# manuelruder/fast-artistic-videos

Measured on AMD Instinct MI355X. Metric: stylized frames/sec @1280x720, per-frame hot path (mask + warp + assembly + net + deprocess + PNG encode on the GPU) with inputs resident in HBM; file->PNG rate of the product CLI (BASELINE.json's end-to-end) in `end_to_end_fps` / `e2e`, PSNR vs CPU ref in `parity`, higher is better.
Workload: dtype f32

## Files before the change

### fast-artistic-videos_amd/csrc/conv_device.h

```cpp
#pragma once
#include "fav_internal.h"

namespace fav {

typedef float f32x16 __attribute__((ext_vector_type(16)));
typedef float v4f __attribute__((ext_vector_type(4)));
typedef int v4i __attribute__((ext_vector_type(4)));
typedef float v2f __attribute__((ext_vector_type(2)));

constexpr int BM = CONV_BM;
constexpr int BK = 32;
constexpr int LDSS = 36;
constexpr int SK_GRID = 512;

__device__ __forceinline__ int xcd_linear_block()
{
    const int nwg = gridDim.x, q = nwg >> 3, r = nwg & 7, xcd = blockIdx.x & 7, idx = blockIdx.x >> 3;
    return (xcd < r ? xcd * (q + 1) : r * (q + 1) + (xcd - r) * q) + idx;
}

__device__ __forceinline__ void store16_wt(void* p, v4f v)
{
    asm volatile("global_store_dwordx4 %0, %1, off sc1" ::"v"(p), "v"(v) : "memory");
}

__device__ __forceinline__ float2 merge_wave_stats(const float2* st, const int* wn, int NW, int pitch, int c, int* n_out)
{
    int n = 0; float s = 0.f;
    for (int w = 0; w < NW; ++w) { n += wn[w]; s += (float)wn[w] * st[w * pitch + c].x; }
    const float mean = n ? s / (float)n : 0.f;
    float m2 = 0.f;
    for (int w = 0; w < NW; ++w) { const float d = st[w * pitch + c].x - mean; m2 += st[w * pitch + c].y + (float)wn[w] * d * d; }
    *n_out = n;
    return make_float2(mean, m2);
}

__device__ __forceinline__ float4 affine4_lo(float4 v, const float* sc, const float* sh, float lo)
{
    const float4 s = *reinterpret_cast<const float4*>(sc);
    const float4 b = *reinterpret_cast<const float4*>(sh);
    v.x = fmaxf(fmaf(v.x, s.x, b.x), lo); v.y = fmaxf(fmaf(v.y, s.y, b.y), lo);
    v.z = fmaxf(fmaf(v.z, s.z, b.z), lo); v.w = fmaxf(fmaf(v.w, s.w, b.w), lo);
    return v;
}

__device__ __forceinline__ float4 affine4(float4 v, const float* sc, const float* sh, int relu)
{
    const float4 s = *reinterpret_cast<const float4*>(sc);
    const float4 b = *reinterpret_cast<const float4*>(sh);
    v.x = fmaf(v.x, s.x, b.x); v.y = fmaf(v.y, s.y, b.y); v.z = fmaf(v.z, s.z, b.z); v.w = fmaf(v.w, s.w, b.w);
    if (relu) { v.x = fmaxf(v.x, 0.f); v.y = fmaxf(v.y, 0.f); v.z = fmaxf(v.z, 0.f); v.w = fmaxf(v.w, 0.f); }
    return v;
// ... 4 lines not shown
```

### fast-artistic-videos_amd/csrc/fav_internal.h

```cpp
#pragma once
#include <hip/hip_runtime.h>
#include <cstdarg>
#include <cstdint>
#include <cstdio>
#include <exception>
#include <new>
#include <string>
#include <vector>

#include "../../include/fav.h"

#include <cstdlib>
inline const char* diag_env(const char* name)
{
#ifdef FAV_DIAG
    return getenv(name);
#else
    (void)name;
    return nullptr;
#endif
}

namespace fav {

// ... 71 lines not shown
__host__ __device__ inline bool stat_acc_poisoned(long long hi_sum, long long hi_squares)
{
    return hi_sum >= STAT_NONFINITE / 2 || hi_sum <= -(STAT_NONFINITE / 2) || hi_squares >= STAT_NONFINITE / 2 || hi_squares <= -(STAT_NONFINITE / 2);
}

struct ConvLaunch {
    const float* in = nullptr;
    int IH = 0, IW = 0;
    int IWp = 0;
    int ups = 0;
    int stuff = 0;
    int CIN = 0;
    Affine pre;
    const float* wgt = nullptr;
    const unsigned short* wgt16 = nullptr;
    const float* bias = nullptr;
    int COUT = 0, COUTp = 0;
    int KH = 0, KW = 0, stride = 1, pad = 0;
    int Kpad = 0;
    int OH = 0, OW = 0;
    float* out = nullptr;
    float* partials = nullptr;
    int final_mode = 0;
    float tanh_mul = 1.f;
    float* out_planar = nullptr;
    float* out_raw_nchw = nullptr;
    float* sk_ws = nullptr; unsigned* sk_flags = nullptr; unsigned sk_epoch = 0;
    unsigned* sk_err = nullptr;
    int reserve_cus = 0;
    int no_sk = 0;
    const float* join_skip = nullptr; float* join_out = nullptr; int OWp = 0;
    long long* stat_acc = nullptr;
    float* ks_ws = nullptr; int* ks_cnt = nullptr;
};
inline size_t conv3_wino4_ksplit_bytes() { return (size_t)256 * 2 * 256 * 128 * sizeof(float); }
size_t conv_streamk_workspace_bytes();
int conv_streamk_grid();
constexpr int CONV_BM = 128;
inline int conv_mblocks(int OH, int OW) { return (OH * OW + CONV_BM - 1) / CONV_BM; }
int launch_conv(const ConvLaunch& p, hipStream_t st);
bool conv_c8_eligible(int cin_pitch, int coutp, int k, int stride, int stages, int ups);
int conv_c8_tiles(int OH, int OW);
int launch_conv_c8(const ConvLaunch& p, int* counts, hipStream_t st);
bool conv_c8d_eligible(int cin_pitch, int cin_real, int coutp, int k, int stride, int stages, int ups);
void conv_c8d_pack(const float* w, int cin, int cout, std::vector<float>& out);
int launch_conv_c8d(const ConvLaunch& p, int cin_real, const float* wc8d, int* counts, hipStream_t st);
bool conv3_halo_eligible(int cin_pitch, int coutp, int k, int stride);
int conv3_halo_tiles(int OH, int OW, bool edge_b);
int launch_conv3_halo(const ConvLaunch& p, int* counts, hipStream_t st);
bool conv3s2_eligible(int cin_pitch, int coutp, int k, int stride, int stages, int ups);
int conv3s2_tiles(int OH, int OW);
int launch_conv3s2(const ConvLaunch& p, int* counts, hipStream_t st);
bool conv_fold_eligible(int cin_pitch, int cout, int k, int stride);
bool conv_fold_launchable(int cin_pitch, int k, int pad, int ups, int IH, int IW);
int launch_conv_fold(const ConvLaunch& p, const float* wfold, hipStream_t st);
int conv_first_tiles(int OH, int OW);
int launch_conv_first(const ConvLaunch& p, int cin_real, const float* wpk, int* counts, hipStream_t st);
bool conv_first2d_eligible(int cin_pitch, int cin_real, int coutp, int k, int stride, int stages, int ups);
int conv_first2d_tiles(int OH, int OW);
int launch_conv_first2d(const ConvLaunch& p, int cin_real, const float* wpk, int* counts, hipStream_t st);
bool conv3_wino_eligible(int cin_pitch, int cout, int coutp, int k, int stride, int pad, int stages, int ups);
int conv3_wino_tiles(int OH, int OW);
int launch_conv3_wino(const ConvLaunch& p, const float* wpk, int* counts, hipStream_t st);
bool conv3_wino4_eligible(int cin_pitch, int cout, int coutp, int k, int stride, int pad, int stages, int ups);
int conv3_wino4_tiles(int OH, int OW);
int launch_conv3_wino4(const ConvLaunch& p, const float* wpk, int* counts, hipStream_t st);
// ... 106 lines not shown
```

### fast-artistic-videos_amd/csrc/kernels_first.hip

```cpp
#include <algorithm>
#include <cstdlib>
#include <vector>

#include "fav_internal.h"
#include "conv_device.h"
#include "launch_common.h"
#include "first_pack.h"
#include "first2d_pack.h"

namespace fav {

namespace {

constexpr int F_TH = 8, F_TW = 64;
constexpr int F_HR = F_TH + 8, F_HC = F_TW + 8;
constexpr int F_HALF = F_HC / 2;
constexpr int F_RP = F_HC;
constexpr int F_CPL = F_HR * F_RP;
constexpr int F_HP = F_HR * F_HC;
constexpr int F_NH = (F_HP + 511) / 512;

struct FirstArgs {
    const float* in; const float* wpk; const float* bias;
    float* out; float2* partials; int* counts;
    int IH, IW, IWp, COUT, pad, OH, OW, tiles_x, tiles_y;
    int COUTP, groups;
    long long* dbg = nullptr;
};

__device__ __forceinline__ float2 merge_rows(const float2* st, const int* wn, int c, int* n_out)
{
    int n = 0; float s = 0.f;
    for (int w = 0; w < 8; ++w) { n += wn[w]; s += (float)wn[w] * st[w * 32 + c].x; }
    const float mean = n ? s / (float)n : 0.f;
    float m2 = 0.f;
    for (int w = 0; w < 8; ++w) { const float d = st[w * 32 + c].x - mean; m2 += st[w * 32 + c].y + (float)wn[w] * d * d; }
    *n_out = n;
    return make_float2(mean, m2);
}

constexpr int f_off(int e) { return (e & 1) * F_HALF + (e >> 1); }

template <int CR>
__global__ __launch_bounds__(512, 2) void conv_first_kernel(const FirstArgs p)
{
    constexpr int NCC = (CR / 2) * 27, NJ = NCC + 14, LAST = CR - 1;
    extern __shared__ __attribute__((aligned(16))) float smem[];
    float* const Ws = smem;
    float* const Hs = Ws + 4 * NJ * 64;
    float* const red = Hs + CR * F_CPL;
    const int t = threadIdx.x, lane = t & 63, wave = t >> 6;

    for (int e = t; e < 4 * NJ * 16; e += 512) *reinterpret_cast<v4f*>(Ws + e * 4) = *reinterpret_cast<const v4f*>(p.wpk + e * 4);

    const int ntiles = p.tiles_x * p.tiles_y;
    float4 hlo[F_NH], hhi[F_NH];
#define FL_LOAD_HALO(tile_)                                                                         \
    {                                                                                               \
        const int ty_ = (tile_) / p.tiles_x, tx_ = (tile_) - ty_ * p.tiles_x;                       \
// ... 146 lines not shown
    }
#undef FL_LOAD_HALO
#undef FL_STORE_HALO
}

template <int CR>
int launch_first_t(const FirstArgs& a, int reserve_cus, hipStream_t st)
{
    const size_t lds = (size_t)(4 * conv_first_pairs(CR) * 64 + CR * F_CPL + 8 * 64 + 8) * sizeof(float);
    static PerDevice cache; int cus;
    FAV_HIP(launch_cus(cache, &cus, conv_first_kernel<CR>));
    const int tiles = a.tiles_x * a.tiles_y;
    const int grid = persistent_slots(cus, reserve_cus);
    hipLaunchKernelGGL((conv_first_kernel<CR>), dim3(tiles < grid ? tiles : grid), dim3(512), lds, st, a);
    FAV_LAUNCH_CHECK("conv_first_kernel");
    return FAV_OK;
}


constexpr int G_TH = 16, G_TW = 32;
constexpr int G_HR = G_TH + 8, G_HC = G_TW + 8;
constexpr int G_CPL = G_HR * G_HC + 16;
constexpr int G_HP = G_HR * G_HC;
constexpr int G_NH = (G_HP + 511) / 512;

template <int CR, bool WIDE = false>
__global__ __launch_bounds__(512, 2) void conv_first2d_kernel(const FirstArgs p)
{
    constexpr int NQ = (9 * CR + 3) / 4;
    extern __shared__ __attribute__((aligned(16))) float smem[];
    float* const Ws = smem;
    float* const Hs = Ws + 16 * NQ * 128;
    float* const red = Hs + CR * G_CPL;
    const int t = threadIdx.x, lane = t & 63, wave = t >> 6;

    const int grp = WIDE ? blockIdx.x % p.groups : 0, tstep = WIDE ? gridDim.x / p.groups : gridDim.x;
    const int PITCH = WIDE ? p.COUTP : 32;
    const float* const wsrc = p.wpk + (WIDE ? (size_t)grp * (16 * NQ * 128) : 0);
    for (int e = t; e < 16 * NQ * 32; e += 512) *reinterpret_cast<v4f*>(Ws + e * 4) = *reinterpret_cast<const v4f*>(wsrc + e * 4);

    const int ntiles = p.tiles_x * p.tiles_y;
    float4 hlo[G_NH], hhi[G_NH];
    const __amdgpu_buffer_rsrc_t irs = __builtin_amdgcn_make_buffer_rsrc(const_cast<float*>(p.in), 0, p.IH * p.IWp * 32, 0x00020000);
#define G_LOAD_HALO(tile_)                                                                          \
    {                                                                                               \
        const bool tv_ = (tile_) < ntiles;                                                          \
        const int ty_ = (tile_) / p.tiles_x, tx_ = (tile_) - ty_ * p.tiles_x;                       \
        _Pragma("unroll") for (int i = 0; i < G_NH; ++i) {                                          \
            const int pix_ = min(t + 512 * i, G_HP - 1), hy_ = pix_ / G_HC, hx_ = pix_ - hy_ * G_HC; \
            const int iy_ = ty_ * G_TH - p.pad + hy_, ix_ = tx_ * G_TW - p.pad + hx_;               \
            const bool v_ = tv_ & ((unsigned)iy_ < (unsigned)p.IH) & ((unsigned)ix_ < (unsigned)p.IW); \
            const int off_ = v_ ? (iy_ * p.IWp + ix_) * 32 : (int)0xFFFFFF00;                       \
            hlo[i] = __builtin_bit_cast(float4, __builtin_amdgcn_raw_buffer_load_b128(irs, off_, 0, 0));          \
            hhi[i] = CR > 4 ? __builtin_bit_cast(float4, __builtin_amdgcn_raw_buffer_load_b128(irs, off_ + 16, 0, 0)) : make_float4(0.f, 0.f, 0.f, 0.f); \
        }                                                                                           \
    }
#define G_STORE_HALO()                                                                              \
    {                                                                                               \
        _Pragma("unroll") for (int i = 0; i < G_NH; ++i) {                                          \
            float* d_ = Hs + min(t + 512 * i, G_HP - 1);                                            \
            const float c_[8] = {hlo[i].x, hlo[i].y, hlo[i].z, hlo[i].w, hhi[i].x, hhi[i].y, hhi[i].z, hhi[i].w}; \
            _Pragma("unroll") for (int c = 0; c < CR; ++c) d_[c * G_CPL] = c_[c];                   \
        }                                                                                           \
    }

    int tile = WIDE ? blockIdx.x / p.groups : blockIdx.x;
    G_LOAD_HALO(tile);
    G_STORE_HALO();

    const int txl = lane & 15, g = lane >> 4;
    int qoff[NQ];
#pragma unroll
    for (int q = 0; q < NQ; ++q) {
        const int idx = 4 * q + g;
        const int c = idx / 9, a = (idx - 9 * c) / 3, b = idx - 9 * c - 3 * a;
        qoff[q] = idx < 9 * CR ? c * G_CPL + 3 * a * G_HC + 3 * b : 0;
    }
    const float* const a_lane = Hs + 2 * wave * G_HC + 2 * txl;
    const float* const b_lo = Ws + lane;
    int hi_words = 8 * NQ * 128;
    asm volatile("" : "+v"(hi_words));
    const float* const b_hi = b_lo + hi_words;
    __syncthreads();

#ifdef FAV_DIAG
    long long dt_[5] = {0, 0, 0, 0, 0}, tq_ = 0; int ntl_ = 0;
#define G_DBG(i_) { if (p.dbg && t == 0) { const long long n_ = wall_clock64(); dt_[i_] += n_ - tq_; tq_ = n_; } }
    if (p.dbg && t == 0) tq_ = wall_clock64();
#else
#define G_DBG(i_)
#endif
    for (; tile < ntiles; tile += tstep) {
        const int nxt = tile + tstep;
        G_LOAD_HALO(nxt);
        G_DBG(0);
        v4f acc[16][2];
#pragma unroll
        for (int ps = 0; ps < 16; ++ps)
#pragma unroll
            for (int nt = 0; nt < 2; ++nt) acc[ps][nt] = v4f{0.f, 0.f, 0.f, 0.f};

        float R[2][16], B[2][8];
#define G_READ_R(set_, q_)                                                                          \
        { const float* rb_ = a_lane + qoff[q_];                                                     \
          _Pragma("unroll") for (int r = 0; r < 4; ++r) _Pragma("unroll") for (int d = 0; d < 4; ++d) R[set_][4 * r + d] = rb_[r * G_HC + d]; }
#define G_READ_B(set_, q_, i_)                                                                      \
        { _Pragma("unroll") for (int j = 0; j < 4; ++j) _Pragma("unroll") for (int nt = 0; nt < 2; ++nt) \
              B[set_][2 * j + nt] = ((i_) < 2 ? b_lo : b_hi)[(((4 * ((i_) & 1) + j) * NQ + (q_)) * 2 + nt) * 64]; }
#define G_FENCE() __builtin_amdgcn_sched_barrier(0)
        G_READ_R(0, 0);
        G_READ_B(0, 0, 0);
#pragma unroll
        for (int q = 0; q < NQ; ++q) {
            if (q + 1 < NQ) { G_READ_R((q + 1) & 1, q + 1); }
#pragma unroll
            for (int i = 0; i < 4; ++i) {
                float L[4], V[4];
                const float* Rq = R[q & 1];
#pragma unroll
                for (int d = 0; d < 4; ++d)
                    L[d] = i == 0 ? Rq[d] - Rq[8 + d] : i == 1 ? Rq[4 + d] + Rq[8 + d] : i == 2 ? Rq[8 + d] - Rq[4 + d] : Rq[4 + d] - Rq[12 + d];
                V[0] = L[0] - L[2]; V[1] = L[1] + L[2]; V[2] = L[2] - L[1]; V[3] = L[1] - L[3];
                const int nset = (4 * q + i + 1) & 1;
                if (i < 3) { G_READ_B(nset, q, i + 1); } else if (q + 1 < NQ) { G_READ_B(nset, q + 1, 0); }
                G_FENCE();
                const float* Bq = B[(4 * q + i) & 1];
// ... 10 lines not shown
#undef G_FENCE
        G_DBG(1);
        __syncthreads();
        G_STORE_HALO();
        G_DBG(2);

        const int ty = tile / p.tiles_x, tx = tile - ty * p.tiles_x;
        const int oy0 = ty * G_TH + 2 * __builtin_amdgcn_readfirstlane(wave), ox0 = tx * G_TW;
        const bool inside = oy0 + 2 <= p.OH && ox0 + G_TW <= p.OW && grp * 32 + 32 <= p.COUT;
        float y[2][4][2][2];
        float sm[2] = {0.f, 0.f};
#pragma unroll
        for (int nt = 0; nt < 2; ++nt) {
            const int ch = grp * 32 + nt * 16 + txl;
            const float bv = p.bias[ch];
            const v2f bv2 = v2f{bv, bv};
#pragma unroll
            for (int rp = 0; rp < 4; rp += 2) {
                v2f Q[4][2];
#pragma unroll
                for (int i = 0; i < 4; ++i) {
                    const v2f m0 = rp ? acc[4 * i][nt].zw : acc[4 * i][nt].xy, m1 = rp ? acc[4 * i + 1][nt].zw : acc[4 * i + 1][nt].xy;
                    const v2f m2 = rp ? acc[4 * i + 2][nt].zw : acc[4 * i + 2][nt].xy, m3 = rp ? acc[4 * i + 3][nt].zw : acc[4 * i + 3][nt].xy;
                    Q[i][0] = (m0 + m1) + m2; Q[i][1] = (m1 - m2) - m3;
                }
#pragma unroll
                for (int b = 0; b < 2; ++b) {
                    const v2f y0 = (Q[0][b] + Q[1][b]) + Q[2][b] + bv2, y1 = (Q[1][b] - Q[2][b]) - Q[3][b] + bv2;
                    y[nt][rp][0][b] = y0.x; y[nt][rp + 1][0][b] = y0.y;
                    y[nt][rp][1][b] = y1.x; y[nt][rp + 1][1][b] = y1.y;
                }
            }
        }
        if (inside) {
            int gq = g, tq = txl;
            asm volatile("" : "+v"(gq), "+v"(tq));
            float* const pb = p.out + ((size_t)oy0 * p.OW + ox0 + 8 * gq) * p.COUT + grp * 32 + tq;
#pragma unroll
            for (int nt = 0; nt < 2; ++nt)
#pragma unroll
                for (int r = 0; r < 4; ++r)
#pragma unroll
                    for (int a = 0; a < 2; ++a)
#pragma unroll
                        for (int b = 0; b < 2; ++b) {
                            pb[((size_t)a * p.OW + 2 * r + b) * p.COUT + nt * 16] = y[nt][r][a][b];
                            sm[nt] += y[nt][r][a][b];
                        }
        } else {
#pragma unroll
            for (int nt = 0; nt < 2; ++nt) {
                const int ch = grp * 32 + nt * 16 + txl;
#pragma unroll
                for (int r = 0; r < 4; ++r)
#pragma unroll
                    for (int a = 0; a < 2; ++a)
#pragma unroll
                        for (int b = 0; b < 2; ++b) {
                            const int oy = oy0 + a, ox = ox0 + 2 * (4 * g + r) + b;
                            if (oy < p.OH && ox < p.OW) {
                                if (ch < p.COUT) p.out[((size_t)oy * p.OW + ox) * p.COUT + ch] = y[nt][r][a][b];
                                sm[nt] += y[nt][r][a][b];
                            }
                        }
            }
        }
// ... 4 lines not shown
            const int nrows = max(0, min(2, p.OH - oy0)), ncols = max(0, min(G_TW, p.OW - ox0));
            const int nw = nrows * ncols;
#pragma unroll
            for (int nt = 0; nt < 2; ++nt) {
                float s = sm[nt];
                s += __shfl_xor(s, 16); s += __shfl_xor(s, 32);
                const float mu = nw ? s / (float)nw : 0.f;
                float qv = 0.f;
                if (inside) {
#pragma unroll
                    for (int r = 0; r < 4; ++r)
#pragma unroll
                        for (int a = 0; a < 2; ++a)
#pragma unroll
                            for (int b = 0; b < 2; ++b) { const float d = y[nt][r][a][b] - mu; qv = fmaf(d, d, qv); }
                } else {
#pragma unroll
                    for (int r = 0; r < 4; ++r)
#pragma unroll
                        for (int a = 0; a < 2; ++a)
#pragma unroll
                            for (int b = 0; b < 2; ++b) {
                                const int oy = oy0 + a, ox = ox0 + 2 * (4 * g + r) + b;
                                const float d = y[nt][r][a][b] - mu;
                                if (oy < p.OH && ox < p.OW) qv = fmaf(d, d, qv);
                            }
                }
                qv += __shfl_xor(qv, 16); qv += __shfl_xor(qv, 32);
                if (lane < 16) st[wave * 32 + nt * 16 + lane] = make_float2(mu, qv);
            }
            if (lane == 0) wn[wave] = nw;
            __syncthreads();
            if (t < 32) {
                int n;
                p.partials[(size_t)tile * PITCH + grp * 32 + t] = merge_rows(st, wn, t, &n);
                if (t == 0 && grp == 0) p.counts[tile] = n;
            }
        }
        __syncthreads();
        G_DBG(4);
#ifdef FAV_DIAG
        ++ntl_;
#endif
    }
#ifdef FAV_DIAG
    if (p.dbg && t == 0) { for (int i = 0; i < 5; ++i) p.dbg[blockIdx.x * 8 + i] = dt_[i]; p.dbg[blockIdx.x * 8 + 5] = ntl_; }
#endif
#undef G_DBG
#undef G_LOAD_HALO
#undef G_STORE_HALO
}

template <int CR, bool WIDE = false>
int launch_first2d_t(const FirstArgs& a, int reserve_cus, hipStream_t st)
{
    const size_t lds = (size_t)(16 * conv_first2d_quads(CR) * 128 + CR * G_CPL + 8 * 64 + 8) * sizeof(float);
    static PerDevice cache; int cus;
    FAV_HIP(launch_cus(cache, &cus, conv_first2d_kernel<CR, WIDE>));
    const int tiles = a.tiles_x * a.tiles_y;
    const int ngrp = WIDE ? a.groups : 1;
    int grid = persistent_slots(cus, reserve_cus);
    grid = std::min(grid, tiles * ngrp);
    if (WIDE) grid = std::max(ngrp, grid / ngrp * ngrp);
#ifdef FAV_DIAG
    static int dbg_n = diag_env("FAV_FIRST_DBG") ? atoi(diag_env("FAV_FIRST_DBG")) : 0;
    static long long* dbuf = nullptr;
    const bool dbg = dbg_n > 0 && --dbg_n == 0;
    FirstArgs ad = a;
    if (dbg) { FAV_HIP(hipMalloc(reinterpret_cast<void**>(&dbuf), 1024 * 8 * 8)); FAV_HIP(hipMemsetAsync(dbuf, 0, 1024 * 8 * 8, st)); ad.dbg = dbuf; }
    hipLaunchKernelGGL((conv_first2d_kernel<CR, WIDE>), dim3(grid), dim3(512), lds, st, ad);
    FAV_LAUNCH_CHECK("conv_first2d_kernel");
    if (dbg) {
        std::vector<long long> hb((size_t)1024 * 8);
        FAV_HIP(hipStreamSynchronize(st)); FAV_HIP(hipMemcpy(hb.data(), dbuf, hb.size() * 8, hipMemcpyDeviceToHost));
        double sum[5] = {0, 0, 0, 0, 0}, nt = 0;
        for (int b = 0; b < grid; ++b) { for (int i = 0; i < 5; ++i) sum[i] += hb[b * 8 + i] * 0.01; nt += hb[b * 8 + 5]; }
        fprintf(stderr, "FIRSTDBG grid=%d tiles=%.0f  per tile (us): halo request %.2f  quads %.2f  barrier + halo to LDS %.2f  transform + stores %.2f  statistics %.2f\n",
                grid, nt, sum[0] / nt, sum[1] / nt, sum[2] / nt, sum[3] / nt, sum[4] / nt);
    }
    return FAV_OK;
#else
    hipLaunchKernelGGL((conv_first2d_kernel<CR, WIDE>), dim3(grid), dim3(512), lds, st, a);
    FAV_LAUNCH_CHECK("conv_first2d_kernel");
    return FAV_OK;
#endif
}

}

int conv_first_tiles(int OH, int OW) { return ((OH + F_TH - 1) / F_TH) * ((OW + F_TW - 1) / F_TW); }

int launch_conv_first(const ConvLaunch& c, int cin_real, const float* wpk, int* counts, hipStream_t st)
{
    FAV_REQUIRE(c.CIN == 8 && (cin_real == 7 || cin_real == 3) && c.COUTp == 32 && c.KH == 9 && c.KW == 9 && c.stride == 1 && c.pre.stages == 0 &&
                c.ups == 0 && !c.final_mode && wpk, "first-layer conv (F(2,3) along x): not eligible");
    FAV_REQUIRE((long long)c.IH * c.IWp * 8 < (1ll << 31), "first-layer conv: bad shape");
    FirstArgs a;
    a.in = c.in; a.wpk = wpk; a.bias = c.bias; a.out = c.out; a.partials = reinterpret_cast<float2*>(c.partials); a.counts = counts;
    a.IH = c.IH; a.IW = c.IW; a.IWp = c.IWp; a.COUT = c.COUT; a.pad = c.pad; a.OH = c.OH; a.OW = c.OW;
    a.tiles_x = (c.OW + F_TW - 1) / F_TW; a.tiles_y = (c.OH + F_TH - 1) / F_TH;
    return cin_real == 7 ? launch_first_t<7>(a, c.reserve_cus, st) : launch_first_t<3>(a, c.reserve_cus, st);
}

bool conv_first2d_eligible(int cin_pitch, int cin_real, int coutp, int k, int stride, int stages, int ups)
{
    return cin_pitch == 8 && (cin_real == 7 || cin_real == 3) && k == 9 && stride == 1 && stages == 0 && ups == 0 && coutp % 32 == 0 && coutp >= 32 && coutp <= 256;
}
int conv_first2d_tiles(int OH, int OW) { return ((OH + G_TH - 1) / G_TH) * ((OW + G_TW - 1) / G_TW); }

int launch_conv_first2d(const ConvLaunch& c, int cin_real, const float* wpk, int* counts, hipStream_t st)
{
    FAV_REQUIRE(conv_first2d_eligible(c.CIN, cin_real, c.COUTp, c.KH, c.stride, c.pre.stages, c.ups) && c.KW == 9 && !c.final_mode && wpk,
                "first-layer conv (F(2x2,3x3) over the nine 3x3 blocks): not eligible");
    FAV_REQUIRE((long long)c.IH * c.IWp * 32 < (1ll << 31) - 512, "first-layer conv: input too large for 32-bit byte offsets");
    FirstArgs a;
    a.in = c.in; a.wpk = wpk; a.bias = c.bias; a.out = c.out; a.partials = reinterpret_cast<float2*>(c.partials); a.counts = counts;
    a.IH = c.IH; a.IW = c.IW; a.IWp = c.IWp; a.COUT = c.COUT; a.pad = c.pad; a.OH = c.OH; a.OW = c.OW;
    a.tiles_x = (c.OW + G_TW - 1) / G_TW; a.tiles_y = (c.OH + G_TH - 1) / G_TH;
    a.COUTP = c.COUTp; a.groups = c.COUTp / 32; a.dbg = nullptr;
    if (a.groups > 1) return cin_real == 7 ? launch_first2d_t<7, true>(a, c.reserve_cus, st) : launch_first2d_t<3, true>(a, c.reserve_cus, st);
    return cin_real == 7 ? launch_first2d_t<7>(a, c.reserve_cus, st) : launch_first2d_t<3>(a, c.reserve_cus, st);
}

}
```

### fast-artistic-videos_amd/csrc/launch_common.h

```cpp
#pragma once
#include <algorithm>
#include <atomic>

#include "fav_internal.h"

namespace fav {

constexpr int MAX_DEVICES = 64;
inline int cur_dev() { int d = 0; (void)hipGetDevice(&d); return (d >= 0 && d < MAX_DEVICES) ? d : 0; }

struct PerDevice {
    std::atomic<int> v[MAX_DEVICES];
    int get(int dv) const { return v[dv].load(std::memory_order_relaxed); }
    void set(int dv, int x) { v[dv].store(x, std::memory_order_relaxed); }
};

template <class... K>
inline hipError_t first_launch_setup(int dv, int* cus, K... kernels)
{
    hipError_t e = hipSuccess;
    for (const void* k : {reinterpret_cast<const void*>(kernels)...})
        if (e == hipSuccess) e = hipFuncSetAttribute(k, hipFuncAttributeMaxDynamicSharedMemorySize, 160 * 1024);
    if (e == hipSuccess) e = hipDeviceGetAttribute(cus, hipDeviceAttributeMultiprocessorCount, dv);
    return e;
}

template <class... K>
inline hipError_t launch_cus(PerDevice& cache, int* cus, K... kernels)
{
    const int dv = cur_dev();
    if ((*cus = cache.get(dv)) != 0) return hipSuccess;
    const hipError_t e = first_launch_setup(dv, cus, kernels...);
    if (e == hipSuccess) cache.set(dv, *cus);
    return e;
}

inline int persistent_slots(int cus, int reserve_cus) { return std::max(1, cus - reserve_cus); }

}
```

### fast-artistic-videos_amd/csrc/net.cpp

```cpp
#include <algorithm>
#include <cmath>
#include <cstdlib>
#include <cstring>
#include <functional>
#include <memory>

#include <mutex>

#include "fav_internal.h"
#include "wino_pack.h"
#include "wino4_pack.h"
#include "up2_pack.h"
#include "s2_pack.h"
#include "first_pack.h"
#include "first2d_pack.h"
#include "fold_pack.h"

using namespace fav;

namespace {

struct DevBuf { void* p = nullptr; size_t bytes = 0; };
struct DevConvW {
    float* wgt = nullptr; float* bias = nullptr; unsigned short* wgt16 = nullptr;
// ... 31 lines not shown
}

void repack_weights(const Layer& L, int cinp, int coutp, int kpad, std::vector<float>& out)
{
    out.assign((size_t)coutp * kpad, 0.f);
    const int taps = L.k * L.k;
    for (int co = 0; co < L.cout; ++co)
        for (int ci = 0; ci < L.cin; ++ci)
            for (int ky = 0; ky < L.k; ++ky)
                for (int kx = 0; kx < L.k; ++kx) {
                    const int tap = ky * L.k + kx;
                    const size_t k = cinp >= 32 ? ((size_t)(ci / 32) * taps + tap) * 32 + ci % 32 : (size_t)tap * cinp + ci;
                    out[(size_t)co * kpad + k] = L.transposed
                        ? L.w[(((size_t)ci * L.cout + co) * L.k + (L.k - 1 - ky)) * L.k + (L.k - 1 - kx)]
                        : L.w[(((size_t)co * L.cin + ci) * L.k + ky) * L.k + kx];
                }
}

struct Tuning {
    bool no_fold = diag_env("FAV_NO_FOLD") != nullptr;
    bool no_c8 = diag_env("FAV_NO_C8") != nullptr;
    bool no_c8d = diag_env("FAV_NO_C8D") != nullptr;
    bool no_first = diag_env("FAV_NO_FIRST") != nullptr;
    bool no_s2w = diag_env("FAV_NO_S2W") != nullptr;
    bool no_up2 = diag_env("FAV_NO_UP2") != nullptr;
    bool no_wino = diag_env("FAV_NO_WINO") != nullptr;
    bool no_h3 = diag_env("FAV_NO_H3") != nullptr;
    bool no_s2 = diag_env("FAV_NO_S2") != nullptr;
    bool first_1d = diag_env("FAV_FIRST_1D") != nullptr;
    bool wino_f2 = diag_env("FAV_WINO_F2") != nullptr;
    bool no_acc_stats = diag_env("FAV_NO_ACC_STATS") != nullptr;
    bool no_lazy_join = diag_env("FAV_NO_LAZY_JOIN") != nullptr;
    bool lazy_join = diag_env("FAV_LAZY_JOIN") != nullptr;
    int side_sk = diag_env("FAV_SIDE_SK") ? atoi(diag_env("FAV_SIDE_SK")) : 0;
};
const Tuning& tuning() { static const Tuning t; return t; }

ConvKernel select_conv(const Layer& L, const DevConvW& d, int stages, int ups, int precision, bool is_final, int IH, int IW, const Tuning& t)
{
    if (is_final) return !t.no_fold && d.packed[CK_FOLD] && conv_fold_launchable(d.cinp, L.k, L.pad, ups, IH, IW) ? CK_FOLD : CK_GENERIC;
    if (L.transposed) return CK_GENERIC;
    const bool c8 = !t.no_c8 && conv_c8_eligible(d.cinp, d.coutp, L.k, L.stride, stages, ups);
    if (!t.no_first && !t.no_c8d) {
        if (c8 && d.packed[CK_FIRST1D] && conv_c8d_eligible(d.cinp, L.cin, d.coutp, L.k, L.stride, stages, ups))
            return d.packed[CK_FIRST2D] && !t.first_1d ? CK_FIRST2D : CK_FIRST1D;
        if (!c8 && d.packed[CK_FIRST2D] && conv_first2d_eligible(d.cinp, L.cin, d.coutp, L.k, L.stride, stages, ups)) return CK_FIRST2D;
    }
    if (d.packed[CK_S2W] && !t.no_s2w && conv3s2w_eligible(d.cinp, L.cout, d.coutp, L.k, L.stride, L.pad, stages, ups)) return CK_S2W;
    if (d.packed[CK_UP2] && precision == 0 && !t.no_up2 &&
        conv3_up2_eligible(d.cinp, L.cout, d.coutp, L.k, L.stride, L.pad, stages, ups)) return CK_UP2;
    if (precision == 0 && !t.no_wino) {
        if (d.packed[CK_WINO4] && conv3_wino4_eligible(d.cinp, L.cout, d.coutp, L.k, L.stride, L.pad, stages, ups)) return CK_WINO4;
        if (d.packed[CK_WINO] && conv3_wino_eligible(d.cinp, L.cout, d.coutp, L.k, L.stride, L.pad, stages, ups)) return CK_WINO;
    }
    if (c8) return !t.no_c8d && d.packed[CK_C8D] && conv_c8d_eligible(d.cinp, L.cin, d.coutp, L.k, L.stride, stages, ups) ? CK_C8D : CK_C8;
    if (!t.no_h3 && conv3_halo_eligible(d.cinp, d.coutp, L.k, L.stride)) return CK_HALO3;
    if (!t.no_s2 && conv3s2_eligible(d.cinp, d.coutp, L.k, L.stride, stages, ups)) return CK_S2HALO;
    return CK_GENERIC;
}

struct ConvFacts { int tiles; bool counts; int id; };
ConvFacts conv_facts(ConvKernel k, int OH, int OW, int coutp, int precision, bool join)
{
    switch (k) {
    case CK_GENERIC: return {conv_mblocks(OH, OW), false, coutp % 128 == 0 ? 128 : (coutp % 64 == 0 ? 64 : 32)};
    case CK_FOLD:    return {0, false, 1};
// ... 148 lines not shown

bool only_tail(const std::vector<Layer>& ls, size_t from, bool& has_tanh, float& mul)
{
    has_tanh = false; mul = 1.f;
    for (size_t i = from; i < ls.size(); ++i) {
        if (ls[i].type == L_TANH) { if (has_tanh) return false; has_tanh = true; }
        else if (ls[i].type == L_MUL) { if (!has_tanh) return false; mul *= ls[i].mul; }
        else if (ls[i].type != L_IDENTITY) return false;
    }
    return true;
}

}

struct fav_net {
    int device = 0;
    std::vector<Layer> layers;
    std::vector<Layer> exec;
    int pad = 0;
    bool pad_folded = false;
    int in_channels = 0;
    long long params = 0;
    std::vector<DevConvW> convs;
    std::vector<DevIN> ins;
    float* ones = nullptr; float* zeros = nullptr;
    float* sk_ws = nullptr; unsigned* sk_flags = nullptr; unsigned sk_epoch = 0;
    float* ks_ws = nullptr; int* ks_cnt = nullptr;
    struct LazyOut { bool active = false; int pitch = 0, rows = 0, shave = 0, conv_index = -1; } lazy;
    unsigned* sk_err_host = nullptr; unsigned* sk_err_dev = nullptr;
    bool shared_device = false;
    int precision = 0;
    int acc_parity = 0;
    bool acc_dirty = false;
    bool branch_tail_acc_ok = false;
    int reserve_cus = 0;
    int curH = 0, curW = 0;
    std::vector<DevBuf> bufs;
    std::vector<void*> slabs; char* slab_cur = nullptr; size_t slab_left = 0;
    size_t cursor = 0, conv_cursor = 0, in_cursor = 0;
    hipStream_t st = nullptr;
    float* stage = nullptr; size_t stage_bytes = 0;
    bool profiling = false;
    struct ProfRec { hipEvent_t a, b; int conv; };
    std::vector<ProfRec> prof_pending;
    std::vector<double> prof_ms, prof_macs; std::vector<int> prof_n, prof_tile;

    ~fav_net()
    {
        (void)hipSetDevice(device);
        (void)hipFree(stage);
        for (auto& c : convs) { (void)hipFree(c.wgt); (void)hipFree(c.bias); (void)hipFree(c.wgt16); for (float* p : c.packed) (void)hipFree(p); }
        for (auto& i : ins) { (void)hipFree(i.gamma); (void)hipFree(i.beta); (void)hipFree(i.scale); (void)hipFree(i.shift); (void)hipFree(i.acc); }
        for (void* sp : slabs) (void)hipFree(sp);
        (void)hipFree(ones); (void)hipFree(zeros); (void)hipFree(sk_ws); (void)hipFree(sk_flags); (void)hipFree(ks_ws); (void)hipFree(ks_cnt); if (sk_err_host) (void)hipHostFree(sk_err_host);
    }
    int upload_layers(std::vector<Layer>& ls, int& chan_pitch, int& maxc);
    int upload();
    int alloc(size_t bytes, float** out);
    int timed_conv(const ConvLaunch& c, int conv_index, const Layer& L, ConvKernel kernel, int* counts);
    int run(std::vector<Layer>& ls, Act& cur, bool top, float* out_planar, float* out_raw);
    bool res_block_is_winograd(const Layer& R, size_t first_conv) const;
    bool acc_stats_ok(const std::vector<Layer>& ls, size_t li) const;
    int forward_padded(const float* in8, int H, int W, float* out_planar, float* out_raw, hipStream_t stream);
    int forward_padded_unordered(const float* in8, int H, int W, float* out_planar, float* out_raw, hipStream_t stream);
    void out_size(int H, int W, int* Ho, int* Wo) const;
};

int fav_net::upload_layers(std::vector<Layer>& ls, int& chan_pitch, int& maxc)
{
    for (Layer& L : ls) {
        if (L.type == L_CONV) {
            convs.emplace_back();
            DevConvW& d = convs.back();
            d.cinp = chan_pitch;
            if (L.cin > chan_pitch || (chan_pitch != 8 && L.cin != chan_pitch)) {
                set_error("network: conv expects %d input channels, producer has %d", L.cin, chan_pitch); return FAV_EFORMAT; }
            if (L.k < 1 || L.stride < 1 || L.pad < 0) { set_error("network: bad convolution geometry"); return FAV_EFORMAT; }
            if ((d.cinp & (d.cinp - 1)) != 0) {
                set_error("network: a convolution with %d input channels is unsupported (channel counts must be powers of two)", d.cinp);
                return FAV_EUNSUPPORTED; }
            d.coutp = (L.cout + 31) / 32 * 32;
            d.kpad = (L.k * L.k * d.cinp + 31) / 32 * 32;
            std::vector<float> w;
            repack_weights(L, d.cinp, d.coutp, d.kpad, w);
            int rc = dev_upload(w, 0, &d.wgt); if (rc) return rc;
            rc = dev_upload(L.b, (size_t)d.coutp, &d.bias); if (rc) return rc;
            if (!L.transposed && conv3_halo_eligible(d.cinp, d.coutp, L.k, L.stride)) {
// ... 41 lines not shown
    return FAV_OK;
}

int fav_net::upload()
{
    FAV_HIP(hipSetDevice(device));
    if (layers.empty()) { set_error("network: empty model"); return FAV_EFORMAT; }
    pad = 0; pad_folded = false;
    if (layers[0].type == L_PAD) {
        const Layer& P = layers[0];
        if (P.pad_mode == 0 && P.pl == P.pr && P.pl == P.pt && P.pl == P.pb) { pad = P.pl; pad_folded = true; }
    }
    in_channels = 0;
    for (const Layer& L : layers) if (L.type == L_CONV) { in_channels = L.cin; break; }
    if (in_channels != 7 && in_channels != 3) {
        set_error("network: first convolution has %d input channels; video models take 7 (models_video.lua:57), image models 3", in_channels);
        return FAV_EUNSUPPORTED; }
    exec = layers;
    int chan0 = 8;
    int real0 = in_channels; bool seen_conv = false;
    int rc = pad_channel_counts(exec, chan0, real0, seen_conv, true); if (rc) return rc;
    int chan = 8, maxc = 8;
    rc = upload_layers(exec, chan, maxc); if (rc) return rc;
    params = count_params(layers);
    std::vector<float> o((size_t)maxc, 1.f), z((size_t)maxc, 0.f);
    rc = dev_upload(o, 0, &ones); if (rc) return rc;
    rc = dev_upload(z, 0, &zeros); if (rc) return rc;
    FAV_HIP(hipMalloc(reinterpret_cast<void**>(&sk_ws), conv_streamk_workspace_bytes()));
    FAV_HIP(hipMalloc(reinterpret_cast<void**>(&sk_flags), conv_streamk_grid() * sizeof(unsigned)));
    FAV_HIP(hipMemset(sk_flags, 0, conv_streamk_grid() * sizeof(unsigned)));
    FAV_HIP(hipMalloc(reinterpret_cast<void**>(&ks_ws), conv3_wino4_ksplit_bytes()));
    FAV_HIP(hipMalloc(reinterpret_cast<void**>(&ks_cnt), 256 * sizeof(int)));
    FAV_HIP(hipMemset(ks_cnt, 0, 256 * sizeof(int)));
    FAV_HIP(hipHostMalloc(reinterpret_cast<void**>(&sk_err_host), sizeof(unsigned), hipHostMallocMapped));
    *sk_err_host = 0;
    FAV_HIP(hipHostGetDevicePointer(reinterpret_cast<void**>(&sk_err_dev), sk_err_host, 0));
    return FAV_OK;
}

int fav_net::alloc(size_t bytes, float** out)
{
    bytes = (bytes + 255) / 256 * 256;
    if (cursor < bufs.size()) {
        if (bufs[cursor].bytes < bytes) { set_error("internal: activation arena mismatch"); return FAV_EINVAL; }
        *out = static_cast<float*>(bufs[cursor++].p);
        return FAV_OK;
    }
    if (slab_left < bytes) {
        const size_t sz = std::max(bytes, (size_t)256 << 20);
        void* sp = nullptr;
        FAV_HIP(hipMalloc(&sp, sz));
        slabs.push_back(sp); slab_cur = static_cast<char*>(sp); slab_left = sz;
    }
    DevBuf b; b.bytes = bytes; b.p = slab_cur;
    slab_cur += bytes; slab_left -= bytes;
    bufs.push_back(b); ++cursor;
    *out = static_cast<float*>(b.p);
    return FAV_OK;
}

int fav_net::timed_conv(const ConvLaunch& c, int conv_index, const Layer& L, ConvKernel kernel, int* counts)
{
    if (c.pre.acc1 != nullptr && kernel != CK_WINO4) { set_error("internal: accumulator-form InstanceNorm in front of a kernel that cannot take it"); return FAV_EINVAL; }
    ConvLaunch cs = c;
    cs.reserve_cus = reserve_cus;
    cs.no_sk = shared_device ? 1 : 0;
    cs.sk_ws = sk_ws; cs.sk_flags = sk_flags; cs.sk_epoch = ++sk_epoch;
    cs.sk_err = sk_err_dev;
    cs.ks_ws = ks_ws; cs.ks_cnt = ks_cnt;
    if (sk_epoch == 0xffffffffu) sk_epoch = 0;
    ConvLaunch cg = cs;
    if (reserve_cus > 0 && tuning().side_sk != 1) cg.no_sk = 1;
    auto go = [&]() { return launch_selected(kernel, cs, cg, convs[conv_index], L.cin, counts, st); };
    char tag[96] = "";
    if (TraceRange::enabled()) snprintf(tag, sizeof tag, "fav:conv%d k%d s%d %d->%d %dx%d", conv_index, L.k, L.stride, L.cin, L.cout, c.OW, c.OH);
    TraceRange tr(tag);
    if (!profiling) return go();
    ProfRec r; r.conv = conv_index;
    FAV_HIP(hipEventCreateWithFlags(&r.a, hipEventDisableSystemFence)); FAV_HIP(hipEventCreateWithFlags(&r.b, hipEventDisableSystemFence));
    FAV_HIP(hipEventRecord(r.a, st));
    int rc = go();
    FAV_HIP(hipEventRecord(r.b, st));
    prof_pending.push_back(r);
    if ((int)prof_ms.size() <= conv_index) { prof_ms.resize(conv_index + 1, 0.0); prof_macs.resize(conv_index + 1, 0.0); prof_n.resize(conv_index + 1, 0); prof_tile.resize(conv_index + 1, 0); }
    prof_macs[conv_index] = (double)c.OH * c.OW * L.cout * L.cin * L.k * L.k;
    prof_tile[conv_index] = conv_facts(kernel, c.OH, c.OW, c.COUTp, precision, c.join_skip != nullptr).id;
    return rc;
}

static int count_convs(const std::vector<Layer>& ls)
{
    int n = 0;
    for (const Layer& l : ls) { if (l.type == L_CONV) ++n; else if (l.type == L_RES) n += count_convs(l.block); }
    return n;
}

bool fav_net::acc_stats_ok(const std::vector<Layer>& ls, size_t li) const
{
    if (tuning().no_acc_stats) return false;
    if (li + 3 >= ls.size() || ls[li + 1].type != L_IN || ls[li + 2].type != L_RELU || ls[li + 3].type != L_CONV) return false;
    if (conv_cursor >= convs.size()) return false;
    const Layer& c2 = ls[li + 3]; const DevConvW& d2 = convs[conv_cursor];
// ... 234 lines not shown

int fav_net::forward_padded(const float* in8, int H, int W, float* out_planar, float* out_raw, hipStream_t stream)
{
    FAV_HIP(hipSetDevice(device));
    DeviceOrder& ord = device_order(device);
    std::lock_guard<std::mutex> order_lock(ord.mu);
    if (ord.valid && ord.last != stream && hipStreamSynchronize(ord.last) != hipSuccess)
        (void)hipGetLastError();
    ord.valid = true; ord.last = stream;
    return forward_padded_unordered(in8, H, W, out_planar, out_raw, stream);
}

int fav_net::forward_padded_unordered(const float* in8, int H, int W, float* out_planar, float* out_raw, hipStream_t stream)
{
    if (sk_err_host && *reinterpret_cast<volatile unsigned*>(sk_err_host)) {
        *sk_err_host = 0;
        shared_device = true;
        set_error("a stream-K hand-off between convolution blocks timed out in an earlier launch of this network: its result was "
                  "wrong (two networks running concurrently on one device? see the concurrency note in fav.h)");
        return FAV_EHIP;
    }
    if (H != curH || W != curW) {
        if (!bufs.empty()) {
            FAV_HIP(hipDeviceSynchronize());
            for (void* sp : slabs) (void)hipFree(sp);
            slabs.clear(); slab_cur = nullptr; slab_left = 0;
            bufs.clear();
        }
        curH = H; curW = W;
    }
    st = stream; cursor = 0; conv_cursor = 0; in_cursor = 0;
    if (acc_dirty) {
        for (DevIN& i : ins) if (i.acc) FAV_HIP(hipMemsetAsync(i.acc, 0, i.acc_bytes, stream));
        acc_dirty = false;
    }
    if (precision == 0 && !tuning().no_acc_stats && !tuning().no_wino) acc_parity ^= 1;
    Act cur;
    cur.data = const_cast<float*>(in8); cur.Hp = H + 2 * pad; cur.Wp = W + 2 * pad; cur.C = 8;
    const int rc = run(exec, cur, true, out_planar, out_raw);
    if (rc) acc_dirty = true;
    return rc;
}

static int finish_create(fav_net* net, fav_net** out)
{
    int rc = net->upload();
    if (rc) { delete net; return rc; }
    *out = net;
    return FAV_OK;
}

extern "C" int fav_net_create(const char* t7_path_host, int device, fav_net** out)
{
    FAV_REQUIRE(t7_path_host && out, "fav_net_create: null argument");
    int rc = ensure_device(); if (rc) return rc;
    FAV_ABI_TRY
    std::unique_ptr<fav_net> net(new fav_net());
    net->device = device;
    rc = t7_parse_model(t7_path_host, net->layers);
    if (rc) return rc;
    return finish_create(net.release(), out);
    FAV_ABI_CATCH("fav_net_create")
}

extern "C" int fav_net_pack_host(const char* t7_path_host, void* blob_host, size_t capacity, size_t* bytes)
{
    FAV_REQUIRE(t7_path_host && bytes, "fav_net_pack_host: null argument");
    FAV_ABI_TRY
// ... 187 lines not shown
```

Measured before the change: 656.0.

## Deal first-layer conv tiles dynamically through an atomic counter

Replaces the static strided tile loop of the non-wide first 2D conv kernel with dynamic tile dealing. One thread per block takes the next tile from a per-conv global atomic counter and hands it to the block through LDS; each block's first tile is still its block index. The counters are double-buffered by frame parity so the other buffer can be zeroed in-kernel without an extra memset, and an env flag brings back static scheduling. This aims to balance load across persistent blocks, at the cost of one atomic per tile and one more counter-state bookkeeping path.

```diff
diff --git a/fast-artistic-videos_amd/csrc/conv_device.h b/fast-artistic-videos_amd/csrc/conv_device.h
--- a/fast-artistic-videos_amd/csrc/conv_device.h
+++ b/fast-artistic-videos_amd/csrc/conv_device.h
@@ -18,6 +18,9 @@
     const int nwg = gridDim.x, q = nwg >> 3, r = nwg & 7, xcd = blockIdx.x & 7, idx = blockIdx.x >> 3;
     return (xcd < r ? xcd * (q + 1) : r * (q + 1) + (xcd - r) * q) + idx;
 }
+
+__device__ __forceinline__ int tile_ask(int* cnt) { return __hip_atomic_fetch_add(cnt, 1, __ATOMIC_RELAXED, __HIP_MEMORY_SCOPE_AGENT); }
+__device__ __forceinline__ int tile_of(int answer) { return (int)gridDim.x + answer; }
 
 __device__ __forceinline__ void store16_wt(void* p, v4f v)
 {
diff --git a/fast-artistic-videos_amd/csrc/fav_internal.h b/fast-artistic-videos_amd/csrc/fav_internal.h
--- a/fast-artistic-videos_amd/csrc/fav_internal.h
+++ b/fast-artistic-videos_amd/csrc/fav_internal.h
@@ -127,6 +127,7 @@
     const float* join_skip = nullptr; float* join_out = nullptr; int OWp = 0;
     long long* stat_acc = nullptr;
     float* ks_ws = nullptr; int* ks_cnt = nullptr;
+    int* tile_cnt = nullptr; int* tile_cnt_zero = nullptr;
 };
 inline size_t conv3_wino4_ksplit_bytes() { return (size_t)256 * 2 * 256 * 128 * sizeof(float); }
 size_t conv_streamk_workspace_bytes();
diff --git a/fast-artistic-videos_amd/csrc/kernels_first.hip b/fast-artistic-videos_amd/csrc/kernels_first.hip
--- a/fast-artistic-videos_amd/csrc/kernels_first.hip
+++ b/fast-artistic-videos_amd/csrc/kernels_first.hip
@@ -25,6 +25,7 @@
     float* out; float2* partials; int* counts;
     int IH, IW, IWp, COUT, pad, OH, OW, tiles_x, tiles_y;
     int COUTP, groups;
+    int* cnt = nullptr; int* cnt_zero = nullptr;
     long long* dbg = nullptr;
 };
 
@@ -237,7 +238,13 @@
     float* const Ws = smem;
     float* const Hs = Ws + 16 * NQ * 128;
     float* const red = Hs + CR * G_CPL;
+    int* const tks = reinterpret_cast<int*>(red + 8 * 64 + 8);
     const int t = threadIdx.x, lane = t & 63, wave = t >> 6;
+
+    const bool deal = !WIDE && p.cnt != nullptr;
+    const bool dealer = deal && t == 0;
+    int tk0 = 0;
+    if (dealer) { tk0 = tile_ask(p.cnt); if (blockIdx.x == 0) *p.cnt_zero = 0; }
 
     const int grp = WIDE ? blockIdx.x % p.groups : 0, tstep = WIDE ? gridDim.x / p.groups : gridDim.x;
     const int PITCH = WIDE ? p.COUTP : 32;
@@ -272,6 +279,7 @@
     int tile = WIDE ? blockIdx.x / p.groups : blockIdx.x;
     G_LOAD_HALO(tile);
     G_STORE_HALO();
+    if (dealer) *tks = tile_of(tk0);
 
     const int txl = lane & 15, g = lane >> 4;
     int qoff[NQ];
@@ -295,8 +303,8 @@
 #else
 #define G_DBG(i_)
 #endif
-    for (; tile < ntiles; tile += tstep) {
-        const int nxt = tile + tstep;
+    int nxt = deal ? __builtin_amdgcn_readfirstlane(*tks) : tile + tstep;
+    while (tile < ntiles) {
         G_LOAD_HALO(nxt);
         G_DBG(0);
         v4f acc[16][2];
@@ -373,6 +381,8 @@
                 }
             }
         }
+        int tk = 0;
+        if (dealer && nxt < ntiles) tk = tile_ask(p.cnt);
         if (inside) {
             int gq = g, tq = txl;
             asm volatile("" : "+v"(gq), "+v"(tq));
@@ -443,16 +453,19 @@
             if (lane == 0) wn[wave] = nw;
             __syncthreads();
             if (t < 32) {
-                int n;
-                p.partials[(size_t)tile * PITCH + grp * 32 + t] = merge_rows(st, wn, t, &n);
+                int n, tc = t;
+                asm volatile("" : "+v"(tc));
+                p.partials[(size_t)tile * PITCH + grp * 32 + tc] = merge_rows(st, wn, t, &n);
                 if (t == 0 && grp == 0) p.counts[tile] = n;
             }
         }
+        if (dealer) *tks = nxt < ntiles ? tile_of(tk) : ntiles;
         __syncthreads();
         G_DBG(4);
 #ifdef FAV_DIAG
         ++ntl_;
 #endif
+        tile = nxt; nxt = deal ? __builtin_amdgcn_readfirstlane(*tks) : nxt + tstep;
     }
 #ifdef FAV_DIAG
     if (p.dbg && t == 0) { for (int i = 0; i < 5; ++i) p.dbg[blockIdx.x * 8 + i] = dt_[i]; p.dbg[blockIdx.x * 8 + 5] = ntl_; }
@@ -465,12 +478,12 @@
 template <int CR, bool WIDE = false>
 int launch_first2d_t(const FirstArgs& a, int reserve_cus, hipStream_t st)
 {
-    const size_t lds = (size_t)(16 * conv_first2d_quads(CR) * 128 + CR * G_CPL + 8 * 64 + 8) * sizeof(float);
+    const size_t lds = (size_t)(16 * conv_first2d_quads(CR) * 128 + CR * G_CPL + 8 * 64 + 16) * sizeof(float);
     static PerDevice cache; int cus;
     FAV_HIP(launch_cus(cache, &cus, conv_first2d_kernel<CR, WIDE>));
     const int tiles = a.tiles_x * a.tiles_y;
     const int ngrp = WIDE ? a.groups : 1;
-    int grid = persistent_slots(cus, reserve_cus);
+    int grid = dealt_slots(cus, reserve_cus);
     grid = std::min(grid, tiles * ngrp);
     if (WIDE) grid = std::max(ngrp, grid / ngrp * ngrp);
 #ifdef FAV_DIAG
@@ -529,6 +542,7 @@
     a.IH = c.IH; a.IW = c.IW; a.IWp = c.IWp; a.COUT = c.COUT; a.pad = c.pad; a.OH = c.OH; a.OW = c.OW;
     a.tiles_x = (c.OW + G_TW - 1) / G_TW; a.tiles_y = (c.OH + G_TH - 1) / G_TH;
     a.COUTP = c.COUTp; a.groups = c.COUTp / 32; a.dbg = nullptr;
+    a.cnt = c.tile_cnt; a.cnt_zero = c.tile_cnt_zero;
     if (a.groups > 1) return cin_real == 7 ? launch_first2d_t<7, true>(a, c.reserve_cus, st) : launch_first2d_t<3, true>(a, c.reserve_cus, st);
     return cin_real == 7 ? launch_first2d_t<7>(a, c.reserve_cus, st) : launch_first2d_t<3>(a, c.reserve_cus, st);
 }
diff --git a/fast-artistic-videos_amd/csrc/launch_common.h b/fast-artistic-videos_amd/csrc/launch_common.h
--- a/fast-artistic-videos_amd/csrc/launch_common.h
+++ b/fast-artistic-videos_amd/csrc/launch_common.h
@@ -37,4 +37,11 @@
 
 inline int persistent_slots(int cus, int reserve_cus) { return std::max(1, cus - reserve_cus); }
 
+inline int dealt_slots(int cus, int reserve_cus)
+{
+    static const int cap = diag_env("FAV_PERSIST_GRID") ? std::max(0, atoi(diag_env("FAV_PERSIST_GRID"))) : 0;
+    const int slots = persistent_slots(cus, reserve_cus);
+    return cap > 0 ? std::min(cap, slots) : slots;
 }
+
+}
diff --git a/fast-artistic-videos_amd/csrc/net.cpp b/fast-artistic-videos_amd/csrc/net.cpp
--- a/fast-artistic-videos_amd/csrc/net.cpp
+++ b/fast-artistic-videos_amd/csrc/net.cpp
@@ -87,6 +87,7 @@
     bool no_acc_stats = diag_env("FAV_NO_ACC_STATS") != nullptr;
     bool no_lazy_join = diag_env("FAV_NO_LAZY_JOIN") != nullptr;
     bool lazy_join = diag_env("FAV_LAZY_JOIN") != nullptr;
+    bool static_tiles = diag_env("FAV_STATIC_TILES") != nullptr;
     int side_sk = diag_env("FAV_SIDE_SK") ? atoi(diag_env("FAV_SIDE_SK")) : 0;
 };
 const Tuning& tuning() { static const Tuning t; return t; }
@@ -301,6 +302,7 @@
     int precision = 0;
     int acc_parity = 0;
     bool acc_dirty = false;
+    int* tile_cnt = nullptr; int tile_parity = 0;
     bool branch_tail_acc_ok = false;
     int reserve_cus = 0;
     int curH = 0, curW = 0;
@@ -321,7 +323,7 @@
         for (auto& c : convs) { (void)hipFree(c.wgt); (void)hipFree(c.bias); (void)hipFree(c.wgt16); for (float* p : c.packed) (void)hipFree(p); }
         for (auto& i : ins) { (void)hipFree(i.gamma); (void)hipFree(i.beta); (void)hipFree(i.scale); (void)hipFree(i.shift); (void)hipFree(i.acc); }
         for (void* sp : slabs) (void)hipFree(sp);
-        (void)hipFree(ones); (void)hipFree(zeros); (void)hipFree(sk_ws); (void)hipFree(sk_flags); (void)hipFree(ks_ws); (void)hipFree(ks_cnt); if (sk_err_host) (void)hipHostFree(sk_err_host);
+        (void)hipFree(ones); (void)hipFree(zeros); (void)hipFree(sk_ws); (void)hipFree(sk_flags); (void)hipFree(ks_ws); (void)hipFree(ks_cnt); (void)hipFree(tile_cnt); if (sk_err_host) (void)hipHostFree(sk_err_host);
     }
     int upload_layers(std::vector<Layer>& ls, int& chan_pitch, int& maxc);
     int upload();
@@ -429,6 +431,8 @@
     FAV_HIP(hipMalloc(reinterpret_cast<void**>(&ks_ws), conv3_wino4_ksplit_bytes()));
     FAV_HIP(hipMalloc(reinterpret_cast<void**>(&ks_cnt), 256 * sizeof(int)));
     FAV_HIP(hipMemset(ks_cnt, 0, 256 * sizeof(int)));
+    FAV_HIP(hipMalloc(reinterpret_cast<void**>(&tile_cnt), 2 * convs.size() * sizeof(int)));
+    FAV_HIP(hipMemset(tile_cnt, 0, 2 * convs.size() * sizeof(int)));
     FAV_HIP(hipHostMalloc(reinterpret_cast<void**>(&sk_err_host), sizeof(unsigned), hipHostMallocMapped));
     *sk_err_host = 0;
     FAV_HIP(hipHostGetDevicePointer(reinterpret_cast<void**>(&sk_err_dev), sk_err_host, 0));
@@ -465,6 +469,10 @@
     cs.sk_ws = sk_ws; cs.sk_flags = sk_flags; cs.sk_epoch = ++sk_epoch;
     cs.sk_err = sk_err_dev;
     cs.ks_ws = ks_ws; cs.ks_cnt = ks_cnt;
+    if (!tuning().static_tiles) {
+        cs.tile_cnt = tile_cnt + (size_t)tile_parity * convs.size() + conv_index;
+        cs.tile_cnt_zero = tile_cnt + (size_t)(tile_parity ^ 1) * convs.size() + conv_index;
+    }
     if (sk_epoch == 0xffffffffu) sk_epoch = 0;
     ConvLaunch cg = cs;
     if (reserve_cus > 0 && tuning().side_sk != 1) cg.no_sk = 1;
@@ -765,8 +773,10 @@
     st = stream; cursor = 0; conv_cursor = 0; in_cursor = 0;
     if (acc_dirty) {
         for (DevIN& i : ins) if (i.acc) FAV_HIP(hipMemsetAsync(i.acc, 0, i.acc_bytes, stream));
+        FAV_HIP(hipMemsetAsync(tile_cnt, 0, 2 * convs.size() * sizeof(int), stream));
         acc_dirty = false;
     }
+    tile_parity ^= 1;
     if (precision == 0 && !tuning().no_acc_stats && !tuning().no_wino) acc_parity ^= 1;
     Act cur;
     cur.data = const_cast<float*>(in8); cur.Hp = H + 2 * pad; cur.Wp = W + 2 * pad; cur.C = 8;
```

Result: no change. 655.4 (-0.1%).
